# PJLab-ADG/DetZero

Measured on AMD Instinct MI355X. Metric: LiDAR frames/sec (160k pts, 0.1m voxels), higher is better.
Workload: dtype f32 as f16 pairs (hi+lo, 22-bit significand; 3 f16 MFMA per product, f32 accumulate)

## Files before the change

### detzero_amd/csrc/common.h

```cpp
#pragma once
#include <hip/hip_runtime.h>
#include <stdint.h>
#include <stdio.h>

#include "../../include/detzero_hip.h"

namespace dz {

void set_error(const char *fmt, ...);

#define DZ_CHECK_ARG(cond, ...)                 \
    do {                                        \
        if (!(cond)) {                          \
            dz::set_error(__VA_ARGS__);         \
            return DZ_ERR_INVALID;              \
        }                                       \
    } while (0)

#define DZ_HIP(expr)                                                                     \
    do {                                                                                 \
        hipError_t _e = (expr);                                                          \
        if (_e != hipSuccess) {                                                          \
            dz::set_error("%s failed: %s (%s:%d)", #expr, hipGetErrorString(_e), __FILE__, __LINE__); \
            return DZ_ERR_HIP;                                                           \
        }                                                                                \
    } while (0)

#define DZ_LAUNCH_CHECK()                                                                \
    do {                                                                                 \
        hipError_t _e = hipGetLastError();                                               \
        if (_e != hipSuccess) {                                                          \
            dz::set_error("kernel launch failed: %s (%s:%d)", hipGetErrorString(_e), __FILE__, __LINE__); \
            return DZ_ERR_HIP;                                                           \
        }                                                                                \
    } while (0)

static inline int ceil_div(long a, long b) { return (int)((a + b - 1) / b); }

static inline int tile_masks_words(int cap) { return (cap / 32 + 1 + 3) & ~3; }
static inline size_t align_up(size_t x, size_t a) { return (x + a - 1) / a * a; }

static inline int stream_grid(long work_items, int block) {
    long g = (work_items + block - 1) / block;
    if (g < 1) g = 1;
    if (g > 2048) g = 2048;
    return (int)g;
}

constexpr int DZ_MAX_DEVICES = 32;
struct PerDeviceFlags { bool v[DZ_MAX_DEVICES] = {}; };
static inline int reserve_lds(const void *kernel, int bytes, PerDeviceFlags &done, const char *who) {
    int dev = 0;
    if (hipGetDevice(&dev) != hipSuccess) { set_error("%s: hipGetDevice failed", who); return DZ_ERR_HIP; }
    if (dev >= 0 && dev < DZ_MAX_DEVICES && done.v[dev]) return DZ_OK;
    if (hipFuncSetAttribute(kernel, hipFuncAttributeMaxDynamicSharedMemorySize, bytes) != hipSuccess) {
        set_error("%s: cannot reserve %d bytes of LDS on device %d", who, bytes, dev);
        return DZ_ERR_HIP;
    }
    if (dev >= 0 && dev < DZ_MAX_DEVICES) done.v[dev] = true;
    return DZ_OK;
}
static inline int device_cus() {
    static int cus[DZ_MAX_DEVICES] = {};
// ... 85 lines not shown
```

### detzero_amd/csrc/conv3x3_h.hip

```cpp
#include "hgemm.h"

namespace dz {

constexpr int C3_TW = 32, C3_KC = 32;
constexpr int C3_ROW_U4 = C3_KC / 4 + 1;
constexpr int C3_PXW = C3_TW + 2;
constexpr int C3_NS = 3;
using v2u = __attribute__((ext_vector_type(2))) unsigned int;

constexpr int C3_NT = 512;
template <int BC>
struct C3Cfg {
    static constexpr int PT = 2;
    static constexpr int WC = BC >= 64 ? 2 : 1;
    static constexpr int WP = C3_NT / 64 / WC;
    static constexpr int TH = WP * PT;
    static constexpr int CT = BC / (32 * WC);
    static constexpr int PXH = TH + 2, PX_ROWS = C3_PXW * PXH, PX_PIECES = PX_ROWS * (C3_KC / 4);
    static constexpr int PXPT = (PX_PIECES + C3_NT - 1) / C3_NT;
    static constexpr int W_PIECES = BC * (C3_KC / 4);
    static constexpr int WPT = (W_PIECES + C3_NT - 1) / C3_NT;
    static constexpr int W_U4 = BC * C3_ROW_U4;
    static constexpr int LDS_MAIN_BYTES = (PX_ROWS * C3_ROW_U4 + 2 * W_U4) * 16;
    static constexpr int SG = 4;
// ... 21 lines not shown
    const int ntn = p.cout_pad / BC, nty = ny;
    const int *const tlist = p.in_tiles;
    const int npx = tlist ? tlist[0] : p.batch * tiles_x * tiles_y;
    const int xcd = blockIdx.x & 7, jloc = blockIdx.x >> 3, nj = gridDim.x >> 3;
    const int grp = (pair0 + jloc % nty) / ntn;
    const int n0 = ((pair0 + jloc % nty) % ntn) * BC;
    const int per_xcd = (npx + 7) >> 3;
    const int band_lo = xcd * per_xcd, band_hi = min(npx, band_lo + per_xcd);
    const int tstep = nj / nty;
    int tile = band_lo + jloc / nty;
    if (tstep == 0 || tile >= band_hi) return;

    const srsrc_t prsrc = make_srsrc(p.in, in_bytes);
    const srsrc_t crsrc = make_srsrc(p.w, w_bytes);
    int x0, y0, b;
    auto tile_id = [&](int t) {
        if (!tlist) return t;
        const int *ptr = tlist + 2 + t;
        int id;
        asm volatile("s_load_dword %0, %1, 0x0\n\ts_waitcnt lgkmcnt(0)" : "=&s"(id) : "s"(ptr) : "memory");
        return id;
    };
    auto tile_origin = [&](int t, int &ox, int &oy, int &ob) {
        ox = (t % tiles_x) * C3_TW;
        oy = ((t / tiles_x) % tiles_y) * C3_TH;
        ob = t / (tiles_x * tiles_y);
    };
    struct TileGeo { unsigned int base; int rows, cols; };
    auto tile_geo = [&](int t) {
        int ox, oy, ob;
        tile_origin(t, ox, oy, ob);
        TileGeo g;
        if constexpr (SPARSE) g.base = (unsigned int)((ob * p.in_hp + oy + p.in_off) * p.in_wp + ox + p.in_off);
        else g.base = (unsigned int)((((long)(ob * p.in_hp + oy + p.in_off) * p.in_wp + ox + p.in_off) * p.in_cstride + p.in_coff + grp * p.cin) * 4);
        g.rows = p.in_hp - (oy + p.in_off);
        g.cols = p.in_wp - (ox + p.in_off);
        return g;
    };
    int id_cur = tile_id(tile), id_next = id_cur;
    TileGeo geo = tile_geo(id_cur), geo_next = geo;
    const int prow = tid / (C3_KC / 4), pq = tid % (C3_KC / 4);
    bool has_next = tile + tstep < band_hi;
    unsigned int cvoff[WPT];
#pragma unroll
    for (int i = 0; i < WPT; ++i) {
        const int idx = tid + i * C3_NT;
// ... 360 lines not shown
```

### detzero_amd/csrc/pair16.hip

```cpp
#include "hgemm.h"

namespace dz {

template <class M>
__global__ void k_pair16_from_f32(const float *__restrict__ src, long rows, int c_src, int c_dst, uint4 *__restrict__ dst) {
    const int groups = c_dst / 8;
    const long total = rows * groups;
    for (long idx = (long)blockIdx.x * blockDim.x + threadIdx.x; idx < total; idx += (long)gridDim.x * blockDim.x) {
        const long r = idx / groups;
        const int g = (int)(idx % groups);
        float v[8];
#pragma unroll
        for (int e = 0; e < 8; ++e) v[e] = (g * 8 + e < c_src) ? src[r * c_src + g * 8 + e] : 0.f;
        const float a[4] = {v[0], v[1], v[2], v[3]}, b[4] = {v[4], v[5], v[6], v[7]};
        uint2 h0, l0, h1, l1;
        split4<M>(a, h0, l0);
        split4<M>(b, h1, l1);
        dst[idx * 2] = make_uint4(h0.x, h0.y, h1.x, h1.y);
        dst[idx * 2 + 1] = make_uint4(l0.x, l0.y, l1.x, l1.y);
    }
}

template <class M>
__global__ void k_pair16_to_f32(const uint4 *__restrict__ src, long rows, int c, float *__restrict__ dst) {
// ... 85 lines not shown
        bev[idx * 2 + 1] = zip(l0, l1);
    }
}

__global__ __launch_bounds__(256) void k_bev_row_index(const uint32_t *__restrict__ bitmap, const uint32_t *__restrict__ prefix, LevelGeom lg, int pad,
                                                       int feat_rows, int2 *__restrict__ idx) {
    const int hp = lg.h + 2 * pad, wp = lg.w + 2 * pad;
    const long total = (long)lg.b * hp * wp;
    for (long pix = (long)blockIdx.x * blockDim.x + threadIdx.x; pix < total; pix += (long)gridDim.x * blockDim.x) {
        const int xp = (int)(pix % wp), yp = (int)((pix / wp) % hp), b = (int)(pix / ((long)wp * hp));
        const int x = xp - pad, y = yp - pad;
        int r0 = -1, r1 = -1;
        if ((unsigned)x < (unsigned)lg.w && (unsigned)y < (unsigned)lg.h) {
            r0 = bitmap_find(bitmap, prefix, lg.key(b, 0, y, x));
            r1 = bitmap_find(bitmap, prefix, lg.key(b, 1, y, x));
            if (r0 >= feat_rows) r0 = -1;
            if (r1 >= feat_rows) r1 = -1;
        }
        idx[pix] = make_int2(r0, r1);
    }
}

constexpr int BEV_DCAP = 8;
__global__ __launch_bounds__(256) void k_bev_tile_mind(const int2 *__restrict__ idx, int batch, int hp, int wp, int ho, int wo, int tiles_y, int tiles_x,
                                                       unsigned char *__restrict__ mind) {
    constexpr int R = BEV_DCAP - 1, SH = 8 + 2 * R, SW = 32 + 2 * R;
    __shared__ unsigned char occ[SH][SW + 2];
    __shared__ int tile_min;
    const int t = blockIdx.x;
    const int tx = t % tiles_x, ty = (t / tiles_x) % tiles_y, b = t / (tiles_x * tiles_y);
    const int y0 = ty * 8 - R, x0 = tx * 32 - R;
    if (threadIdx.x == 0) tile_min = BEV_DCAP;
    for (int k = threadIdx.x; k < SH * SW; k += 256) {
        const int ry = k / SW, rx = k - ry * SW;
        const int y = y0 + ry, x = x0 + rx;
        unsigned char o = 0;
        if ((unsigned)y < (unsigned)ho && (unsigned)x < (unsigned)wo) {
            const int2 v = idx[((size_t)b * hp + y + 1) * wp + x + 1];
            o = (v.x >= 0 || v.y >= 0) ? 1 : 0;
        }
        occ[ry][rx] = o;
    }
    __syncthreads();
    const int py = threadIdx.x >> 5, px = threadIdx.x & 31;
    int d = BEV_DCAP;
    if (ty * 8 + py < ho && tx * 32 + px < wo) {
        const int cy = py + R, cx = px + R;
        if (occ[cy][cx]) d = 0;
        else {
            for (int r = 1; r <= R && d == BEV_DCAP; ++r) {
                bool hit = false;
                for (int k = -r; k <= r; ++k)
                    hit |= occ[cy - r][cx + k] | occ[cy + r][cx + k] | occ[cy + k][cx - r] | occ[cy + k][cx + r];
                if (hit) d = r;
            }
        }
    }
    atomicMin(&tile_min, d);
    __syncthreads();
    if (threadIdx.x == 0) mind[t] = (unsigned char)tile_min;
}

__global__ __launch_bounds__(1024) void k_bev_tile_compact(const unsigned char *__restrict__ mind, int n, int *__restrict__ lists, int stride) {
    __shared__ int part[1024];
    const int tid = threadIdx.x, need = (int)blockIdx.x + 2;
    int *const list = lists + (size_t)blockIdx.x * stride;
    const int per = (n + 1023) / 1024, lo = min(n, tid * per), hi = min(n, lo + per);
    int c = 0;
    for (int i = lo; i < hi; ++i) c += mind[i] < need;
    part[tid] = c;
    __syncthreads();
    for (int d = 1; d < 1024; d <<= 1) {
        const int v = tid >= d ? part[tid - d] : 0;
        __syncthreads();
        part[tid] += v;
        __syncthreads();
    }
    const int total = part[1023];
    int occ = part[tid] - c, emp = lo - occ;
    for (int i = lo; i < hi; ++i) {
        if (mind[i] < need) list[2 + occ++] = i;
        else list[2 + total + emp++] = i;
    }
    if (tid == 0) { list[0] = total; list[1] = n - total; }
}

template <class M>
__global__ __launch_bounds__(256) void k_bev_fill_tiles(const int *__restrict__ list, int tiles_y, int tiles_x, int ho, int wo, const float *__restrict__ shift,
                                                        int relu, int cout, float *__restrict__ out, int out_hp, int out_wp, int out_cstride, int out_coff,
                                                        const float *__restrict__ zero_resp) {
    const int n_occ = list[0], n_emp = list[1];
    if ((int)blockIdx.x >= n_emp) return;
    const int t = list[2 + n_occ + blockIdx.x];
    const int tx = t % tiles_x, ty = (t / tiles_x) % tiles_y, b = t / (tiles_x * tiles_y);
    const int groups = cout / 8;
    for (int k = threadIdx.x; k < 8 * 32 * groups; k += 256) {
        const int g = k % groups, px = k / groups, r = px / 32, c = px % 32;
        const int y = ty * 8 + r, x = tx * 32 + c;
        if (y >= ho || x >= wo) continue;
        uint4 *dst = reinterpret_cast<uint4 *>(out + (((size_t)b * out_hp + y + 1) * out_wp + x + 1) * out_cstride + out_coff + g * 8);
        if (zero_resp) {
            const uint4 *src = reinterpret_cast<const uint4 *>(zero_resp + (((size_t)(y + 1)) * out_wp + x + 1) * cout + g * 8);
            dst[0] = src[0];
            dst[1] = src[1];
            continue;
        }
        float v0[4], v1[4];
#pragma unroll
        for (int e = 0; e < 4; ++e) {
            const float a = shift ? shift[g * 8 + e] : 0.f, bb = shift ? shift[g * 8 + 4 + e] : 0.f;
            v0[e] = relu ? fmaxf(a, 0.f) : a;
            v1[e] = relu ? fmaxf(bb, 0.f) : bb;
        }
        uint2 h0, l0, h1, l1;
        split4<M>(v0, h0, l0);
        split4<M>(v1, h1, l1);
        dst[0] = make_uint4(h0.x, h0.y, h1.x, h1.y);
        dst[1] = make_uint4(l0.x, l0.y, l1.x, l1.y);
    }
}

}

using namespace dz;

extern "C" {

size_t dz_bev_tile_list_words(int batch, int ho, int wo) { return (size_t)batch * ceil_div(ho, 8) * ceil_div(wo, 32) + 2; }

int dz_bev_tile_list(const int *idx, int batch, int hp, int wp, int ho, int wo, int nlists, int *lists, unsigned char *mind_ws, void *stream_) {
    hipStream_t stream = (hipStream_t)stream_;
    DZ_CHECK_ARG(idx && lists && mind_ws && batch > 0 && ho > 0 && wo > 0 && hp >= ho + 2 && wp >= wo + 2 && nlists >= 1 && nlists < BEV_DCAP,
                 "dz_bev_tile_list: bad argument (1 <= nlists <= %d)", BEV_DCAP - 1);
    const int ty = ceil_div(ho, 8), tx = ceil_div(wo, 32), n = batch * ty * tx;
    hipLaunchKernelGGL(k_bev_tile_mind, dim3(n), dim3(256), 0, stream, reinterpret_cast<const int2 *>(idx), batch, hp, wp, ho, wo, ty, tx, mind_ws);
    hipLaunchKernelGGL(k_bev_tile_compact, dim3(nlists), dim3(1024), 0, stream, mind_ws, n, lists, (int)dz_bev_tile_list_words(batch, ho, wo));
    DZ_LAUNCH_CHECK();
    return DZ_OK;
}

int dz_bev_fill_empty_tiles(const int *list, int batch, int ho, int wo, const float *shift, int relu, int cout, float *out, int out_hp, int out_wp,
                            int out_cstride, int out_coff, const float *zero_resp, int math, void *stream_) {
    hipStream_t stream = (hipStream_t)stream_;
    DZ_CHECK_ARG(list && out && batch > 0 && ho > 0 && wo > 0 && cout > 0 && cout % 8 == 0 && out_cstride % 8 == 0 && out_coff % 8 == 0 &&
                 out_hp >= ho + 2 && out_wp >= wo + 2, "dz_bev_fill_empty_tiles: bad argument");
    DZ_CHECK_ARG(math == DZ_MATH_F16X2 || math == DZ_MATH_BF16X2 || math == DZ_MATH_F16, "dz_bev_fill_empty_tiles: math %d is not a split mode", math);
    const int ty = ceil_div(ho, 8), tx = ceil_div(wo, 32), n = batch * ty * tx;
    if (math == DZ_MATH_BF16X2)
        hipLaunchKernelGGL(k_bev_fill_tiles<MathBF16>, dim3(n), dim3(256), 0, stream, list, ty, tx, ho, wo, shift, relu, cout, out, out_hp, out_wp, out_cstride,
                           out_coff, zero_resp);
    else
        hipLaunchKernelGGL(k_bev_fill_tiles<MathF16>, dim3(n), dim3(256), 0, stream, list, ty, tx, ho, wo, shift, relu, cout, out, out_hp, out_wp, out_cstride,
                           out_coff, zero_resp);
    DZ_LAUNCH_CHECK();
    return DZ_OK;
}

int dz_bev_row_index(const uint32_t *bitmap, const uint32_t *prefix, int batch, int d, int h, int w, int layout, int pad, int feat_rows, int *idx,
                     void *stream_) {
    hipStream_t stream = (hipStream_t)stream_;
    DZ_CHECK_ARG(bitmap && prefix && idx && batch > 0 && h > 0 && w > 0 && pad >= 0 && feat_rows >= 0, "dz_bev_row_index: bad argument");
    if (d != 2) { set_error("dz_bev_row_index: %d z slabs (the sparse-input convolution reads exactly 2)", d); return DZ_ERR_UNSUPPORTED; }
    DZ_CHECK_ARG(layout == DZ_LAYOUT_LINEAR || layout == DZ_LAYOUT_BRICK, "dz_bev_row_index: bad layout %d", layout);
    const LevelGeom lg = make_level(batch, d, h, w, layout);
    const long total = (long)batch * (h + 2 * pad) * (w + 2 * pad);
    hipLaunchKernelGGL(k_bev_row_index, dim3(stream_grid(total, 256)), dim3(256), 0, stream, bitmap, prefix, lg, pad, feat_rows, reinterpret_cast<int2 *>(idx));
    DZ_LAUNCH_CHECK();
    return DZ_OK;
}

int dz_pair16_from_f32(const float *src, long rows, int c_src, int c_dst, int math, float *dst, void *stream_) {
    hipStream_t stream = (hipStream_t)stream_;
    DZ_CHECK_ARG(rows >= 0 && c_src >= 1 && c_dst >= c_src && c_dst % 8 == 0, "dz_pair16_from_f32: bad sizes");
    DZ_CHECK_ARG(math == DZ_MATH_F16X2 || math == DZ_MATH_BF16X2, "dz_pair16_from_f32: math %d is not a split mode", math);
    if (rows == 0) return DZ_OK;
    DZ_CHECK_ARG(src && dst, "dz_pair16_from_f32: null pointer");
// ... 72 lines not shown
```

### detzero_amd/det_modules.py

```python
import collections
import contextlib
import os
from functools import partial

import numpy as np
import torch
import torch.nn as nn

from . import ops, range_audit
from .lib import DetZeroHipError
from .range_audit import RangeAudit

PACKED_TABLES = bool(os.environ.get('DZ_TUNE_PACKED_TABLES'))

K3, S1, P1 = (3, 3, 3), (1, 1, 1), (1, 1, 1)


def _inference_only(module):
    if module.training:
        raise DetZeroHipError('%s: only the inference path is implemented on the HIP backend '
                              '(call .eval()); training is out of scope' % type(module).__name__)


def fold_bn(bn, conv_bias=None):
# ... 795 lines not shown
                CACHE_GEN[0] += 1
        if torch.cuda.is_current_stream_capturing():
            cache.pin(key)
        elif torch.device(dev).type == 'cuda':
            users.setdefault(key, set()).add(torch.cuda.current_stream(dev))
        return outs

    def _level_convs(self, li, lvl, x, xh, xw, xc, batch, dev, sparse_in=None, out_last=None):
        convs = lvl['convs']
        bufs = None
        tiles = zero = None
        audit = range_audit.active()
        e_in, e_mid = self._e('encoded'), self._e('spatial_features_2d')
        if sparse_in is not None and li == 0 and SKIP_EMPTY_TILES:
            nl = min(len(convs), 6) if all(cv['stride'] == 1 for cv in convs) else 1
            key = ('zero_resp', xh, xw, int(self.math), str(dev), int(batch), e_in, e_mid)
            if nl > 1 and key not in lvl and torch.cuda.is_current_stream_capturing():
                nl = 1
                if not getattr(self, '_warned_capture_nl1', False):
                    self._warned_capture_nl1 = True
                    import warnings
                    warnings.warn('BaseBEVBackbone: graph capture of a %d-frame pass without an eager pass of the same size before it - empty tiles '
                                  'are skipped at the first layer only (run one eager pass first to skip them in all six)' % batch)
            tiles = ops.bev_tile_list(sparse_in[1], xh, xw, nl)
            zero = self._zero_response(lvl, xh, xw, sparse_in[0].shape[1], dev, batch) if nl > 1 else None
        for ci, cv in enumerate(convs):
            s = cv['stride']
            oh, ow = (xh + 2 - 3) // s + 1, (xw + 2 - 3) // s + 1
            if bufs is None:
                bufs = [bordered_zeros('bev2d.l%d.%d' % (li, k), (batch, oh + 2, ow + 2, cv['cout']), dev) for k in range(2)]
            y = out_last if (out_last is not None and ci == len(convs) - 1) else bufs[ci % 2]
            if sparse_in is not None and li == 0 and ci == 0:
                rows, ridx = sparse_in
                wz, scz, shz = self._p(cv, e_in, e_mid, key='w_zmajor')
                conv_layer(rows, (xh + 2, xw + 2), wz, scz, shz, True, y, (oh + 2, ow + 2),
                           cin=cv['cin'], in_cstride=xc, ksize=3, stride=s, in_off=0, out_cstride=cv['cout'],
                           out_d=(1, 1), ho=oh, wo=ow, batch=batch, math=self.math, in_rowidx=ridx, in_row_channels=rows.shape[1],
                           in_rows=rows.shape[0], in_tiles=tiles[0] if tiles is not None else None)
                if tiles is not None:
                    ops.bev_fill_empty_tiles(tiles[0], batch, oh, ow, shz, True, cv['cout'], y, self.math)
            else:
                tl = tiles[ci] if (tiles is not None and ci < tiles.shape[0]) else None
                wc, scc, shc = self._p(cv, e_in if (li == 0 and ci == 0) else e_mid, e_mid)
                conv_layer(x, (xh + 2, xw + 2), wc, scc, shc, True, y, (oh + 2, ow + 2),
                           cin=cv['cin'], in_cstride=xc, ksize=3, stride=s, in_off=0, out_cstride=cv['cout'],
                           out_d=(1, 1), ho=oh, wo=ow, batch=batch, math=self.math, in_tiles=tl, w_limb3=self._l3(cv))
                if tl is not None:
# ... 430 lines not shown
```

### detzero_amd/lib.py

```python
import ctypes
import os

import torch

_HERE = os.path.dirname(os.path.abspath(__file__))
LIB_PATH = os.path.join(_HERE, 'libdetzero_hip.so')


ERR_INVALID, ERR_WORKSPACE, ERR_HIP, ERR_UNSUPPORTED = -1, -2, -3, -4


class DetZeroHipError(RuntimeError):
    pass


c_int, c_float, c_size_t, c_void_p, c_double = ctypes.c_int, ctypes.c_float, ctypes.c_size_t, ctypes.c_void_p, ctypes.c_double
c_longlong = ctypes.c_longlong
_I3 = c_int * 3
_F3 = c_float * 3
_F6 = c_float * 6
_I8 = c_int * 8


class Conv2dDesc(ctypes.Structure):
# ... 92 lines not shown
                                        c_void_p, c_void_p, c_void_p, c_int, c_void_p, c_int, c_int, c_void_p]),
    'dz_spconv_tiles_variant': (ctypes.c_char_p, [c_int, c_int]),
    'dz_spconv_x_tile_rows': (c_int, [c_int, c_int]),
    'dz_spconv_x_window_rows': (c_int, [c_int, c_int]),
    'dz_spconv_x_windows_words': (c_size_t, [c_int, c_int]),
    'dz_spconv_x_windows': (c_int, [c_void_p, c_int, c_void_p, c_int, c_void_p, c_void_p, c_void_p, c_void_p]),
    'dz_build_neighbors_packed_x': (c_int, [c_void_p, c_void_p, c_int, c_void_p, c_void_p, c_int, c_int, c_int, c_int, c_void_p, c_void_p, c_int,
                                            c_void_p, c_void_p, c_void_p, c_void_p]),
    'dz_spconv_forward_split_x': (c_int, [c_void_p, c_int, c_int, c_void_p, c_void_p, c_void_p, c_int, c_int, c_void_p, c_void_p, c_void_p, c_void_p,
                                          c_void_p, c_int, c_void_p, c_int, c_int, c_void_p]),
    'dz_spconv_x_variant': (ctypes.c_char_p, [c_int, c_int]),
    'dz_spconv_forward_x_f32': (c_int, [c_void_p, c_int, c_int, c_void_p, c_void_p, c_void_p, c_int, c_int, c_void_p, c_void_p, c_void_p, c_void_p,
                                        c_void_p, c_int, c_void_p, c_int, c_void_p]),
    'dz_spconv_x_f32_window_rows': (c_int, [c_int, c_int]),
    'dz_spconv_x_f32_variant': (ctypes.c_char_p, [c_int, c_int]),
    'dz_spconv_forward_x_limb3': (c_int, [c_void_p, c_int, c_int, c_void_p, c_void_p, c_void_p, c_int, c_int, c_void_p, c_void_p, c_void_p, c_void_p,
                                          c_void_p, c_int, c_void_p, c_int, c_void_p]),
    'dz_spconv_x_limb3_window_rows': (c_int, [c_int, c_int]),
    'dz_spconv_x_limb3_variant': (ctypes.c_char_p, [c_int, c_int]),
    'dz_spconv_forward_limb3': (c_int, [c_void_p, c_int, c_int, c_void_p, c_void_p, c_int, c_int, c_void_p, c_void_p, c_void_p, c_void_p,
                                        c_void_p, c_int, c_void_p, c_int, c_void_p]),
    'dz_spconv_limb3_tile_rows': (c_int, [c_int, c_int]),
    'dz_spconv_limb3_variant': (ctypes.c_char_p, [c_int, c_int]),
    'dz_bev_tile_list_words': (c_size_t, [c_int, c_int, c_int]),
    'dz_bev_tile_list': (c_int, [c_void_p, c_int, c_int, c_int, c_int, c_int, c_int, c_void_p, c_void_p, c_void_p]),
    'dz_bev_fill_empty_tiles': (c_int, [c_void_p, c_int, c_int, c_int, c_void_p, c_int, c_int, c_void_p, c_int, c_int, c_int, c_int, c_void_p, c_int, c_void_p]),
    'dz_bev_row_index': (c_int, [c_void_p, c_void_p, c_int, c_int, c_int, c_int, c_int, c_int, c_int, c_void_p, c_void_p]),
    'dz_sparse_to_bev_split': (c_int, [c_void_p, c_void_p, c_void_p, c_int, c_int, c_int, c_int, c_int, c_int, c_void_p,
                                       c_void_p]),
    'dz_sparse_to_bev_split_dense': (c_int, [c_void_p, c_int, c_void_p, c_void_p, c_int, c_int, c_int, c_int, c_int, c_int, c_int, c_void_p,
                                             c_void_p]),
    'dz_conv2d_forward_split': (c_int, [ctypes.POINTER(Conv2dDesc), c_int, c_int, c_void_p]),
    'dz_conv2d_variant_split': (ctypes.c_char_p, [ctypes.POINTER(Conv2dDesc), c_int]),
    'dz_conv3x3_limb3_forward': (c_int, [ctypes.POINTER(Conv2dDesc), c_void_p]),
    'dz_conv3x3_limb3_supported': (c_int, [ctypes.POINTER(Conv2dDesc)]),
    'dz_conv3x3_limb3_variant': (ctypes.c_char_p, [ctypes.POINTER(Conv2dDesc)]),
    'dz_spconv_variant_split': (ctypes.c_char_p, [c_int, c_int]),
    'dz_spconv_variant_split_arm': (ctypes.c_char_p, [c_int, c_int, c_int, c_int, c_size_t]),
    'dz_spconv_variant_split_packed': (ctypes.c_char_p, [c_int, c_int]),
    'dz_xattn_folded_supported': (c_int, [c_int, c_int, c_int]),
    'dz_xattn_folded_workspace_bytes': (ctypes.c_size_t, [c_int, c_int]),
    'dz_xattn_folded': (c_int, [c_void_p] * 6 + [c_int] * 5 + [ctypes.c_float, c_void_p, ctypes.c_size_t, c_void_p, c_void_p]),
    'dz_roi_bev_features': (c_int, [c_void_p, c_int, c_void_p, ctypes.c_long, ctypes.c_long, c_int, c_int, c_int] + [ctypes.c_float] * 4 + [c_int, c_void_p, c_void_p]),
    'dz_linear_splitk_workspace_bytes': (ctypes.c_size_t, [c_int, c_int, c_int]),
    'dz_linear_forward_splitk': (c_int, [c_void_p, c_int, c_int, c_int, c_void_p, c_int, c_int, c_void_p, c_void_p, c_int, c_void_p, c_int, c_int, c_void_p,
                                         ctypes.c_size_t, c_void_p]),
    'dz_mha_core_split': (c_int, [c_void_p, c_void_p, c_void_p, c_void_p, c_int, c_int, c_int, c_int, ctypes.c_float, c_void_p, c_int, c_void_p]),
    'dz_pdv_sa_pool_supported': (c_int, [c_int] * 7),
    'dz_pdv_sa_pool': (c_int, [c_void_p, c_int, c_int, c_void_p, c_void_p, c_int, c_void_p, c_void_p, c_int, c_void_p, c_void_p, c_int,
# ... 146 lines not shown
```

### detzero_amd/ops.py

```python
import ctypes
import os
from typing import Callable, NamedTuple, Optional

import numpy as np
import torch

from . import lib as L


def _dev():
    return torch.device('cuda', torch.cuda.current_device())


def _ws(nbytes):
    return torch.empty((max(int(nbytes), 256),), dtype=torch.uint8, device=_dev())


def grid_size_of(pc_range, voxel_size):
    r = np.asarray(pc_range, dtype=np.float32)
    return np.round((r[3:6] - r[0:3]) / np.array(voxel_size)).astype(np.int64)


def voxelize_hard_nosync(points, pc_range, voxel_size, max_points, max_voxels, xy_range_mask=False):
    lib = L.load()
# ... 427 lines not shown
        launch()
    else:
        m = out_level.num_active()
        pairs = table_pairs(nbr, m)
        flops = 2.0 * pairs * cin * cout
        n_in = in_level.num_active() if in_level is not None else m
        nbytes = 4.0 * (n_in * cin + m * cout + nbr.kvol * cin * cout + (m * cout if residual is not None else 0)) + 8.0 * pairs
        PROFILER.wrap(route.variant(cin, cout).decode(), flops, nbytes, launch)
    return out


def bev_row_index(level, feat_rows, pad=1):
    lib = L.load()
    d, h, w = level.shape
    idx = torch.empty((level.batch, h + 2 * pad, w + 2 * pad, 2), dtype=torch.int32, device=level.coords.device)
    rc = lib.dz_bev_row_index(L.ptr(level.bitmap), L.ptr(level.prefix), level.batch, d, h, w, level.layout, pad, int(feat_rows), L.ptr(idx), L.stream())
    L.check(rc, 'dz_bev_row_index')
    return idx


def bev_tile_list(ridx, ho, wo, nlists=1):
    lib = L.load()
    b, hp, wp, _ = ridx.shape
    n = lib.dz_bev_tile_list_words(b, int(ho), int(wo))
    lst = torch.empty((int(nlists), n), dtype=torch.int32, device=ridx.device)
    ws = torch.empty((n,), dtype=torch.uint8, device=ridx.device)
    L.check(lib.dz_bev_tile_list(L.ptr(ridx), b, hp, wp, int(ho), int(wo), int(nlists), L.ptr(lst), L.ptr(ws), L.stream()), 'dz_bev_tile_list')
    return lst


def bev_fill_empty_tiles(tiles, batch, ho, wo, shift, relu, cout, out, math, zero_resp=None):
    lib = L.load()
    L.check(lib.dz_bev_fill_empty_tiles(L.ptr(tiles), int(batch), int(ho), int(wo), L.ptr(shift), 1 if relu else 0, int(cout), L.ptr(out), out.shape[1],
                                        out.shape[2], out.shape[3], 0, L.ptr(zero_resp), int(math), L.stream()), 'dz_bev_fill_empty_tiles')


BEV_DENSE = not os.environ.get('DZ_BEV_SCATTER')


def sparse_to_bev(feats, level, c, pad=1, out=None, math=0):
    lib = L.load()
    d, h, w = level.shape
    if out is None:
        out = torch.empty((level.batch, h + 2 * pad, w + 2 * pad, c * d), dtype=torch.float32, device=feats.device)
    if math and d == 2 and c % 8 == 0 and BEV_DENSE:
        rc = lib.dz_sparse_to_bev_split_dense(L.ptr(feats), feats.shape[0], L.ptr(level.bitmap), L.ptr(level.prefix), level.batch, c, d, h, w, level.layout,
                                              pad, L.ptr(out), L.stream())
        L.check(rc, 'dz_sparse_to_bev_split_dense')
        return out
    out.zero_()
    fn = lib.dz_sparse_to_bev_split if math else lib.dz_sparse_to_bev
    rc = fn(L.ptr(feats), L.ptr(level.coords), L.ptr(level.d_m), level.cap, c, d, h, w, pad, L.ptr(out), L.stream())
    L.check(rc, 'dz_sparse_to_bev')
    return out


MATH_MODES = {'f32': 0, 'f16x2': 1, 'bf16x2': 2, 'f16': 3}
# ... 181 lines not shown
def conv2d(desc_kwargs, math=0, out_f32=False, tiles=None, f32_engine=None):
    lib = L.load()
    if f32_engine not in (None,) + DENSE_F32_ENGINES:
        raise L.DetZeroHipError('unknown fp32 dense engine %r (%s)' % (f32_engine, ' | '.join(DENSE_F32_ENGINES)))
    limb3 = f32_engine == 'bf16x3' and not math
    d = _conv2d_desc(desc_kwargs)

    def launch():
        if limb3:
            L.check(lib.dz_conv3x3_limb3_forward(ctypes.byref(d), L.stream()), 'dz_conv3x3_limb3_forward')
        elif math:
            L.check(lib.dz_conv2d_forward_split(ctypes.byref(d), int(math), 1 if out_f32 else 0, L.stream()), 'dz_conv2d_forward_split')
        else:
            L.check(lib.dz_conv2d_forward(ctypes.byref(d), L.stream()), 'dz_conv2d_forward')
    if PROFILER is None:
        launch()
        return
    m = d.batch * d.ho * d.wo
    taps = d.kh * d.kw
    cout = sum(d.g_cout[i] for i in range(d.groups))
    flops = 2.0 * m * taps * d.cin * cout
    nbytes = 4.0 * (m * d.cin * (1 if d.phase_groups else d.groups) + m * cout + taps * d.cin * d.cout_pad * d.groups)
    if tiles is not None:
        n_run, n_skip = (int(v) for v in tiles[:2].tolist())
        share = n_run / float(max(n_run + n_skip, 1))
        flops *= share
        nbytes = 4.0 * (share * (m * d.cin + m * cout) + taps * d.cin * d.cout_pad * d.groups)
    if limb3:
        name = lib.dz_conv3x3_limb3_variant(ctypes.byref(d)).decode()
    else:
        name = (lib.dz_conv2d_variant_split(ctypes.byref(d), 1 if out_f32 else 0) if math else lib.dz_conv2d_variant(ctypes.byref(d))).decode()
    PROFILER.wrap(name, flops, nbytes, launch)


def linear(x, w, scale, shift, relu, cout, out=None, group_shift=None, group_rows=0):
    lib = L.load()
    L.require_cuda(x, w, scale, shift, group_shift)
    rows, cin = x.shape
    cout_pad = w.shape[1]
    if out is None:
        out = torch.empty((rows, cout), dtype=torch.float32, device=x.device)
    rc = lib.dz_linear_forward(L.ptr(x), rows, cin, x.stride(0), L.ptr(w), cout, cout_pad, L.ptr(scale),
                               L.ptr(shift), L.ptr(group_shift), int(group_rows), 1 if relu else 0, L.ptr(out),
                               out.stride(0), L.stream())
    L.check(rc, 'dz_linear_forward')
    return out


# ... 748 lines not shown
```

### include/detzero_hip.h

```cpp
#ifndef DETZERO_HIP_H
#define DETZERO_HIP_H

#include <stddef.h>
#include <stdint.h>

#ifdef __cplusplus
extern "C" {
#endif

#define DZ_OK 0
#define DZ_ERR_INVALID (-1)
#define DZ_ERR_WORKSPACE (-2)
#define DZ_ERR_HIP (-3)
#define DZ_ERR_UNSUPPORTED (-4)

const char *dz_version(void);
const char *dz_last_error(void);
int dz_device_cu_count(void);


size_t dz_voxelize_hard_workspace_bytes(int n, int gx, int gy, int gz, int max_points);
int dz_voxelize_hard(const float *points, int n, int c, const float *h_range6, const float *h_vsize3,
                     const int *h_grid3, int xy_range_mask, int max_points, int max_voxels, float *voxels,
                     int *coords_zyx, int *num_points, int *d_num_voxels, void *ws, size_t ws_bytes,
// ... 118 lines not shown
                                int h, int w, int *nbr_packed, uint32_t *tile_masks, int tile_rows, int *windows, int *nbr_sorted,
                                int *perm, void *stream);
int dz_spconv_forward_split_x(const float *in, int in_rows, int cin, const int *nbr_packed, const int *perm, int *windows, int tile_rows,
                              int cap_out, const int *d_m_out, const float *w, const float *scale, const float *shift,
                              const float *residual, int relu, float *out, int cout, int math, void *stream);
const char *dz_spconv_x_variant(int cin, int cout);
int dz_spconv_forward_x_f32(const float *in, int in_rows, int cin, const int *nbr_packed, const int *perm, int *windows, int tile_rows,
                            int cap_out, const int *d_m_out, const float *w, const float *scale, const float *shift,
                            const float *residual, int relu, float *out, int cout, void *stream);
int dz_spconv_x_f32_window_rows(int cin, int cout);
const char *dz_spconv_x_f32_variant(int cin, int cout);
int dz_spconv_forward_x_limb3(const float *in, int in_rows, int cin, const int *nbr_packed, const int *perm, int *windows, int tile_rows,
                              int cap_out, const int *d_m_out, const float *w, const float *scale, const float *shift,
                              const float *residual, int relu, float *out, int cout, void *stream);
int dz_spconv_x_limb3_window_rows(int cin, int cout);
const char *dz_spconv_x_limb3_variant(int cin, int cout);
int dz_spconv_forward_limb3(const float *in, int in_rows, int cin, const int *nbr, const uint32_t *tile_masks, int kvol, int cap_out,
                            const int *d_m_out, const float *w_limb, const float *scale, const float *shift, const float *residual,
                            int relu, float *out, int cout, void *stream);
int dz_spconv_limb3_tile_rows(int cin, int cout);
const char *dz_spconv_limb3_variant(int cin, int cout);
int dz_bev_row_index(const uint32_t *bitmap, const uint32_t *prefix, int batch, int d, int h, int w, int layout, int pad, int feat_rows,
                     int *idx, void *stream);
size_t dz_bev_tile_list_words(int batch, int ho, int wo);
int dz_bev_tile_list(const int *idx, int batch, int hp, int wp, int ho, int wo, int nlists, int *lists, unsigned char *mind_ws, void *stream);
int dz_bev_fill_empty_tiles(const int *list, int batch, int ho, int wo, const float *shift, int relu, int cout, float *out, int out_hp, int out_wp,
                            int out_cstride, int out_coff, const float *zero_resp, int math, void *stream);
int dz_sparse_to_bev_split(const float *feats, const int *coords, const int *d_m, int cap, int c, int d, int h,
                           int w, int pad, float *bev, void *stream);
int dz_sparse_to_bev_split_dense(const float *feats, int feat_rows, const uint32_t *bitmap, const uint32_t *prefix, int batch, int c,
                                 int d, int h, int w, int layout, int pad, float *bev, void *stream);
int dz_conv2d_forward_split(const dz_conv2d_desc *h_desc, int math, int out_f32, void *stream);
const char *dz_conv2d_variant_split(const dz_conv2d_desc *h_desc, int out_f32);
int dz_conv3x3_limb3_forward(const dz_conv2d_desc *h_desc, void *stream);
int dz_conv3x3_limb3_supported(const dz_conv2d_desc *h_desc);
const char *dz_conv3x3_limb3_variant(const dz_conv2d_desc *h_desc);
int dz_linear_forward_split(const float *x, long rows, int cin, int x_stride, const float *w, int cout, int cout_pad, const float *scale,
                            const float *shift, const float *group_shift, int group_rows, int relu, float *y, int y_stride, int math,
                            int out_f32, int group_max, void *stream);
const char *dz_spconv_variant_split(int cin, int cout);
const char *dz_spconv_variant_split_arm(int cin, int cout, int kvol, int has_tile_masks, size_t nbr_bytes);
const char *dz_spconv_variant_split_packed(int cin, int cout);
int dz_xattn_folded_supported(int lq, int e, int heads);
size_t dz_xattn_folded_workspace_bytes(int b, int lk);
int dz_xattn_folded(const float *q, const float *mem, const uint8_t *key_padding_mask, const float *wk_oi, const float *wv_io, const float *bv,
                    int b, int lq, int lk, int e, int heads, float scale, float *workspace, size_t workspace_bytes, float *out, void *stream);
int dz_mlp_chain_forward(const float *x, long rows, const float *wa, const float *sa, const float *ba, const float *group_shift, int ldg, int group_rows,
                         const float *wb, const float *sb, const float *bb, const float *wk, const float *bk, const float *wv, const float *bv,
                         float *mem, float *k, float *v, int math, void *stream);
int dz_pointnet3_forward(const float *x, long rows, const float *w1, const float *s1, const float *b1, const float *w2, const float *s2,
// ... 214 lines not shown
```

Baseline: 1182.

## Replace fixed BEV tile grid skip with per-band greedy tile cover and span fills

Instead of skipping only fixed 32-wide grid tiles that are empty, each 8-row band is planned with a greedy cover that places 32-wide tiles starting at the first busy column, so fewer conv tiles are launched. The remaining empty gaps are emitted as spans and filled by a persistent grid-stride kernel with deeper vectorized stores. Conv3x3 tiles gain packed (batch, row, x) entries with arbitrary x origins. This adds planning complexity, packing limits on size and width, and a separate grid list for other consumers.

```diff
diff --git a/detzero_amd/csrc/common.h b/detzero_amd/csrc/common.h
--- a/detzero_amd/csrc/common.h
+++ b/detzero_amd/csrc/common.h
@@ -39,6 +39,10 @@
 
 static inline int tile_masks_words(int cap) { return (cap / 32 + 1 + 3) & ~3; }
 static inline size_t align_up(size_t x, size_t a) { return (x + a - 1) / a * a; }
+
+constexpr int TILE_XY_MAX_B = 1 << 10, TILE_XY_MAX_TY = 1 << 9, TILE_XY_MAX_X = 1 << 12;
+__host__ __device__ static inline int tile_xy_pack(int b, int ty, int x) { return (int)(0x80000000u | ((unsigned)b << 21) | ((unsigned)ty << 12) | (unsigned)x); }
+__host__ __device__ static inline void tile_xy_unpack(int e, int &b, int &ty, int &x) { x = e & 0xFFF; ty = (e >> 12) & 0x1FF; b = (e >> 21) & 0x3FF; }
 
 static inline int stream_grid(long work_items, int block) {
     long g = (work_items + block - 1) / block;
diff --git a/detzero_amd/csrc/conv3x3_h.hip b/detzero_amd/csrc/conv3x3_h.hip
--- a/detzero_amd/csrc/conv3x3_h.hip
+++ b/detzero_amd/csrc/conv3x3_h.hip
@@ -67,6 +67,12 @@
         return id;
     };
     auto tile_origin = [&](int t, int &ox, int &oy, int &ob) {
+        if (tlist && t < 0) {
+            int ty;
+            tile_xy_unpack(t, ob, ty, ox);
+            oy = ty * C3_TH;
+            return;
+        }
         ox = (t % tiles_x) * C3_TW;
         oy = ((t / tiles_x) % tiles_y) * C3_TH;
         ob = t / (tiles_x * tiles_y);
diff --git a/detzero_amd/csrc/pair16.hip b/detzero_amd/csrc/pair16.hip
--- a/detzero_amd/csrc/pair16.hip
+++ b/detzero_amd/csrc/pair16.hip
@@ -131,101 +131,164 @@
 }
 
 constexpr int BEV_DCAP = 8;
-__global__ __launch_bounds__(256) void k_bev_tile_mind(const int2 *__restrict__ idx, int batch, int hp, int wp, int ho, int wo, int tiles_y, int tiles_x,
-                                                       unsigned char *__restrict__ mind) {
-    constexpr int R = BEV_DCAP - 1, SH = 8 + 2 * R, SW = 32 + 2 * R;
-    __shared__ unsigned char occ[SH][SW + 2];
-    __shared__ int tile_min;
-    const int t = blockIdx.x;
-    const int tx = t % tiles_x, ty = (t / tiles_x) % tiles_y, b = t / (tiles_x * tiles_y);
-    const int y0 = ty * 8 - R, x0 = tx * 32 - R;
-    if (threadIdx.x == 0) tile_min = BEV_DCAP;
-    for (int k = threadIdx.x; k < SH * SW; k += 256) {
-        const int ry = k / SW, rx = k - ry * SW;
-        const int y = y0 + ry, x = x0 + rx;
-        unsigned char o = 0;
-        if ((unsigned)y < (unsigned)ho && (unsigned)x < (unsigned)wo) {
-            const int2 v = idx[((size_t)b * hp + y + 1) * wp + x + 1];
-            o = (v.x >= 0 || v.y >= 0) ? 1 : 0;
-        }
-        occ[ry][rx] = o;
+constexpr int BEV_MAX_W = 1024;
+static inline __host__ __device__ int bev_slot_words(int tiles_x) { return 3 + tiles_x + tiles_x + 1; }
+
+__global__ __launch_bounds__(256) void k_bev_cover_plan(const int2 *__restrict__ idx, int hp, int wp, int ho, int wo, int tiles_y, int tiles_x, int nl,
+                                                        int *__restrict__ slots) {
+    __shared__ unsigned char vd[BEV_MAX_W];
+    __shared__ unsigned long long busy[BEV_DCAP - 2][BEV_MAX_W / 64];
+    const int tid = threadIdx.x, ty = blockIdx.x % tiles_y, b = blockIdx.x / tiles_y, y0 = ty * 8;
+    for (int k = tid; k < (BEV_DCAP - 2) * (BEV_MAX_W / 64); k += 256) (&busy[0][0])[k] = 0ull;
+    for (int x = tid; x < wo; x += 256) {
+        int v = BEV_DCAP - 1;
+        for (int r = -nl; r < 8 + nl; ++r) {
+            const int y = y0 + r;
+            if ((unsigned)y >= (unsigned)ho) continue;
+            const int2 e = idx[((size_t)b * hp + y + 1) * wp + x + 1];
+            if (e.x >= 0 || e.y >= 0) v = min(v, r < 0 ? -r : r > 7 ? r - 7 : 0);
+        }
+        vd[x] = (unsigned char)v;
     }
     __syncthreads();
-    const int py = threadIdx.x >> 5, px = threadIdx.x & 31;
-    int d = BEV_DCAP;
-    if (ty * 8 + py < ho && tx * 32 + px < wo) {
-        const int cy = py + R, cx = px + R;
-        if (occ[cy][cx]) d = 0;
-        else {
-            for (int r = 1; r <= R && d == BEV_DCAP; ++r) {
-                bool hit = false;
-                for (int k = -r; k <= r; ++k)
-                    hit |= occ[cy - r][cx + k] | occ[cy + r][cx + k] | occ[cy + k][cx - r] | occ[cy + k][cx + r];
-                if (hit) d = r;
+    const int wo64 = (wo + 63) & ~63;
+    for (int l = 1; l <= nl; ++l)
+        for (int x = tid; x < wo64; x += 256) {
+            bool bz = false;
+            if (x < wo)
+                for (int k = max(0, x - l); k <= min(wo - 1, x + l); ++k) bz |= vd[k] <= l;
+            const unsigned long long m = __ballot(bz);
+            if ((tid & 63) == 0) busy[l - 1][x >> 6] = m;
+        }
+    __syncthreads();
+    if (tid >= nl) return;
+    const unsigned long long *const bm = busy[tid];
+    int *const s = slots + ((size_t)blockIdx.x * nl + tid) * bev_slot_words(tiles_x);
+    const int nw = wo64 >> 6;
+    int n = 0, ns = 0, pos = 0;
+    for (;;) {
+        int w = pos >> 6, x = wo;
+        unsigned long long m = bm[w] & (~0ull << (pos & 63));
+        while (!m && ++w < nw) m = bm[w];
+        if (m) x = w * 64 + __ffsll(m) - 1;
+        if (x > pos) s[3 + tiles_x + ns++] = pos | (x << 16);
+        if (x >= wo) break;
+        s[3 + n++] = x;
+        pos = x + 32;
+        if (pos >= wo) break;
+    }
+    unsigned int gm = 0u;
+    for (int tx = 0; tx < tiles_x; ++tx) gm |= (unsigned int)(bm[tx >> 1] >> (32 * (tx & 1))) ? 1u << tx : 0u;
+    s[0] = n;
+    s[1] = ns;
+    s[2] = (int)gm;
+}
+
+__global__ __launch_bounds__(64) void k_bev_cover_compact(const int *__restrict__ slots, int n_bands, int tiles_y, int tiles_x, int nl, int *__restrict__ lists,
+                                                          int stride) {
+    const int lane = threadIdx.x, l = blockIdx.y, first = blockIdx.x * 64, sw = bev_slot_words(tiles_x);
+    auto slot = [&](int i) { return slots + ((size_t)i * nl + l) * sw; };
+    int before[3] = {0, 0, 0}, total[3] = {0, 0, 0};
+    for (int i = lane; i < n_bands; i += 64) {
+        const int *s = slot(i);
+        const int c[3] = {s[0], s[1], (int)__popc((unsigned int)s[2])};
+        for (int k = 0; k < 3; ++k) { total[k] += c[k]; if (i < first) before[k] += c[k]; }
+    }
+    for (int k = 0; k < 3; ++k)
+        for (int d = 32; d >= 1; d >>= 1) { total[k] += __shfl_xor(total[k], d); before[k] += __shfl_xor(before[k], d); }
+    const int me = first + lane;
+    const bool live = me < n_bands;
+    const int *const s = slot(live ? me : 0);
+    const int n = live ? s[0] : 0, ns = live ? s[1] : 0;
+    const unsigned int gm = live ? (unsigned int)s[2] : 0u;
+    int pre[3] = {n, ns, (int)__popc(gm)};
+    for (int k = 0; k < 3; ++k) {
+        for (int d = 1; d < 64; d <<= 1) { const int t = __shfl_up(pre[k], d); if (lane >= d) pre[k] += t; }
+        pre[k] += before[k];
+    }
+    int *const grid = lists + (size_t)l * stride, *const cover = grid + 2 + n_bands * tiles_x;
+    if (blockIdx.x == 0 && lane == 0) {
+        grid[0] = total[2];
+        grid[1] = n_bands * tiles_x - total[2];
+        cover[0] = total[0];
+        cover[1] = total[1];
+    }
+    if (!live) return;
+    const int b = me / tiles_y, ty = me % tiles_y;
+    int *o = cover + 2 + pre[0] - n;
+    for (int k = 0; k < n; ++k) o[k] = tile_xy_pack(b, ty, s[3 + k]);
+    o = cover + 2 + total[0] + 2 * (pre[1] - ns);
+    for (int k = 0; k < ns; ++k) {
+        const int sp = s[3 + tiles_x + k];
+        o[2 * k] = tile_xy_pack(b, ty, sp & 0xFFFF);
+        o[2 * k + 1] = sp >> 16;
+    }
+    int run = pre[2] - (int)__popc(gm);
+    for (int tx = 0; tx < tiles_x; ++tx) {
+        const int id = me * tiles_x + tx;
+        if ((gm >> tx) & 1u) grid[2 + run++] = id;
+        else grid[2 + total[2] + id - run] = id;
+    }
+}
+
+constexpr int FILL_DEPTH = 8;
+template <class M>
+__global__ __launch_bounds__(256) void k_bev_fill_spans(const int *__restrict__ list, int batch, int tiles_y, int tiles_x, int ho, int wo,
+                                                        const float *__restrict__ shift, int relu, int cout, float *__restrict__ out, int out_hp, int out_wp,
+                                                        int out_cstride, int out_coff, const float *__restrict__ zero_resp) {
+    const int n_run = list[0], n_fill = min(list[1], batch * tiles_y * (tiles_x + 1));
+    if (n_fill <= 0) return;
+    const int *const ent = list + 2 + n_run;
+    const bool xy = ent[0] < 0;
+    const int lane = threadIdx.x & 63;
+    const int y8 = blockIdx.x & 7;
+    const int wave = __builtin_amdgcn_readfirstlane((int)((blockIdx.x >> 3) * 4 + (threadIdx.x >> 6))), nwaves = (gridDim.x >> 3) * 4;
+    const int ppp = cout / 4;
+    const int nseg = (wo + 63) / 64;
+    for (int u = wave; u < n_fill * nseg; u += nwaves) {
+        const int i = u / nseg, seg = u - i * nseg;
+        int b, ty, xs, xe;
+        if (xy) {
+            tile_xy_unpack(ent[2 * i], b, ty, xs);
+            xe = ent[2 * i + 1];
+        } else {
+            const int t = ent[i];
+            xs = (t % tiles_x) * 32, xe = min(xs + 32, wo), ty = (t / tiles_x) % tiles_y, b = t / (tiles_x * tiles_y);
+        }
+        const int y = ty * 8 + y8;
+        if ((unsigned)b >= (unsigned)batch || y >= ho || xs < 0 || xe > wo) continue;
+        xs += seg * 64;
+        if (xs >= xe) continue;
+        xe = min(xe, xs + 64);
+        const int np = (xe - xs) * ppp;
+        float *const drow = out + (((size_t)b * out_hp + y + 1) * out_wp + xs + 1) * out_cstride + out_coff;
+        const uint4 *const srow = zero_resp ? reinterpret_cast<const uint4 *>(zero_resp + ((size_t)(y + 1) * out_wp + xs + 1) * cout) : nullptr;
+        for (int p0 = lane; p0 < np; p0 += 64 * FILL_DEPTH) {
+            uint4 v[FILL_DEPTH];
+#pragma unroll
+            for (int k = 0; k < FILL_DEPTH; ++k) {
+                const int p = p0 + 64 * k;
+                if (p >= np) continue;
+                if (srow) { v[k] = srow[p]; continue; }
+                const int g = (p % ppp) >> 1;
+                float v0[4], v1[4];
+#pragma unroll
+                for (int e = 0; e < 4; ++e) {
+                    const float a = shift ? shift[g * 8 + e] : 0.f, bb = shift ? shift[g * 8 + 4 + e] : 0.f;
+                    v0[e] = relu ? fmaxf(a, 0.f) : a;
+                    v1[e] = relu ? fmaxf(bb, 0.f) : bb;
+                }
+                uint2 h0, l0, h1, l1;
+                split4<M>(v0, h0, l0);
+                split4<M>(v1, h1, l1);
+                v[k] = (p & 1) ? make_uint4(l0.x, l0.y, l1.x, l1.y) : make_uint4(h0.x, h0.y, h1.x, h1.y);
             }
-        }
-    }
-    atomicMin(&tile_min, d);
-    __syncthreads();
-    if (threadIdx.x == 0) mind[t] = (unsigned char)tile_min;
-}
-
-__global__ __launch_bounds__(1024) void k_bev_tile_compact(const unsigned char *__restrict__ mind, int n, int *__restrict__ lists, int stride) {
-    __shared__ int part[1024];
-    const int tid = threadIdx.x, need = (int)blockIdx.x + 2;
-    int *const list = lists + (size_t)blockIdx.x * stride;
-    const int per = (n + 1023) / 1024, lo = min(n, tid * per), hi = min(n, lo + per);
-    int c = 0;
-    for (int i = lo; i < hi; ++i) c += mind[i] < need;
-    part[tid] = c;
-    __syncthreads();
-    for (int d = 1; d < 1024; d <<= 1) {
-        const int v = tid >= d ? part[tid - d] : 0;
-        __syncthreads();
-        part[tid] += v;
-        __syncthreads();
-    }
-    const int total = part[1023];
-    int occ = part[tid] - c, emp = lo - occ;
-    for (int i = lo; i < hi; ++i) {
-        if (mind[i] < need) list[2 + occ++] = i;
-        else list[2 + total + emp++] = i;
-    }
-    if (tid == 0) { list[0] = total; list[1] = n - total; }
-}
-
-template <class M>
-__global__ __launch_bounds__(256) void k_bev_fill_tiles(const int *__restrict__ list, int tiles_y, int tiles_x, int ho, int wo, const float *__restrict__ shift,
-                                                        int relu, int cout, float *__restrict__ out, int out_hp, int out_wp, int out_cstride, int out_coff,
-                                                        const float *__restrict__ zero_resp) {
-    const int n_occ = list[0], n_emp = list[1];
-    if ((int)blockIdx.x >= n_emp) return;
-    const int t = list[2 + n_occ + blockIdx.x];
-    const int tx = t % tiles_x, ty = (t / tiles_x) % tiles_y, b = t / (tiles_x * tiles_y);
-    const int groups = cout / 8;
-    for (int k = threadIdx.x; k < 8 * 32 * groups; k += 256) {
-        const int g = k % groups, px = k / groups, r = px / 32, c = px % 32;
-        const int y = ty * 8 + r, x = tx * 32 + c;
-        if (y >= ho || x >= wo) continue;
-        uint4 *dst = reinterpret_cast<uint4 *>(out + (((size_t)b * out_hp + y + 1) * out_wp + x + 1) * out_cstride + out_coff + g * 8);
-        if (zero_resp) {
-            const uint4 *src = reinterpret_cast<const uint4 *>(zero_resp + (((size_t)(y + 1)) * out_wp + x + 1) * cout + g * 8);
-            dst[0] = src[0];
-            dst[1] = src[1];
-            continue;
-        }
-        float v0[4], v1[4];
-#pragma unroll
-        for (int e = 0; e < 4; ++e) {
-            const float a = shift ? shift[g * 8 + e] : 0.f, bb = shift ? shift[g * 8 + 4 + e] : 0.f;
-            v0[e] = relu ? fmaxf(a, 0.f) : a;
-            v1[e] = relu ? fmaxf(bb, 0.f) : bb;
-        }
-        uint2 h0, l0, h1, l1;
-        split4<M>(v0, h0, l0);
-        split4<M>(v1, h1, l1);
-        dst[0] = make_uint4(h0.x, h0.y, h1.x, h1.y);
-        dst[1] = make_uint4(l0.x, l0.y, l1.x, l1.y);
+#pragma unroll
+            for (int k = 0; k < FILL_DEPTH; ++k) {
+                const int p = p0 + 64 * k;
+                if (p < np) *reinterpret_cast<uint4 *>(drow + (size_t)(p / ppp) * out_cstride + (p % ppp) * 4) = v[k];
+            }
+        }
     }
 }
 
@@ -235,32 +298,43 @@
 
 extern "C" {
 
-size_t dz_bev_tile_list_words(int batch, int ho, int wo) { return (size_t)batch * ceil_div(ho, 8) * ceil_div(wo, 32) + 2; }
-
-int dz_bev_tile_list(const int *idx, int batch, int hp, int wp, int ho, int wo, int nlists, int *lists, unsigned char *mind_ws, void *stream_) {
-    hipStream_t stream = (hipStream_t)stream_;
-    DZ_CHECK_ARG(idx && lists && mind_ws && batch > 0 && ho > 0 && wo > 0 && hp >= ho + 2 && wp >= wo + 2 && nlists >= 1 && nlists < BEV_DCAP,
-                 "dz_bev_tile_list: bad argument (1 <= nlists <= %d)", BEV_DCAP - 1);
-    const int ty = ceil_div(ho, 8), tx = ceil_div(wo, 32), n = batch * ty * tx;
-    hipLaunchKernelGGL(k_bev_tile_mind, dim3(n), dim3(256), 0, stream, reinterpret_cast<const int2 *>(idx), batch, hp, wp, ho, wo, ty, tx, mind_ws);
-    hipLaunchKernelGGL(k_bev_tile_compact, dim3(nlists), dim3(1024), 0, stream, mind_ws, n, lists, (int)dz_bev_tile_list_words(batch, ho, wo));
-    DZ_LAUNCH_CHECK();
-    return DZ_OK;
-}
-
-int dz_bev_fill_empty_tiles(const int *list, int batch, int ho, int wo, const float *shift, int relu, int cout, float *out, int out_hp, int out_wp,
-                            int out_cstride, int out_coff, const float *zero_resp, int math, void *stream_) {
+static inline int bev_bands(int batch, int ho) { return batch * ceil_div(ho, 8); }
+size_t dz_bev_tile_cover_offset(int batch, int ho, int wo) { return (size_t)bev_bands(batch, ho) * ceil_div(wo, 32) + 2; }
+size_t dz_bev_tile_cover_words(int batch, int ho, int wo) {
+    const size_t n = bev_bands(batch, ho), tx = ceil_div(wo, 32);
+    return dz_bev_tile_cover_offset(batch, ho, wo) + 2 + n * tx + 2 * n * (tx + 1);
+}
+size_t dz_bev_tile_cover_ws_words(int batch, int ho, int wo, int nlists) { return (size_t)bev_bands(batch, ho) * nlists * bev_slot_words(ceil_div(wo, 32)); }
+
+int dz_bev_tile_cover(const int *idx, int batch, int hp, int wp, int ho, int wo, int nlists, int *lists, int *ws, void *stream_) {
+    hipStream_t stream = (hipStream_t)stream_;
+    DZ_CHECK_ARG(idx && lists && ws && batch > 0 && ho > 0 && wo > 0 && hp >= ho + 2 && wp >= wo + 2 && nlists >= 1 && nlists <= BEV_DCAP - 2,
+                 "dz_bev_tile_cover: bad argument (1 <= nlists <= %d)", BEV_DCAP - 2);
+    const int ty = ceil_div(ho, 8), tx = ceil_div(wo, 32), n = batch * ty;
+    DZ_CHECK_ARG(wo <= BEV_MAX_W && wo <= TILE_XY_MAX_X && ty <= TILE_XY_MAX_TY && batch <= TILE_XY_MAX_B,
+                 "dz_bev_tile_cover: %d frames of %d x %d pixels exceed the list entry (%d frames, %d rows, %d columns)", batch, ho, wo, TILE_XY_MAX_B,
+                 TILE_XY_MAX_TY * 8, BEV_MAX_W);
+    hipLaunchKernelGGL(k_bev_cover_plan, dim3(n), dim3(256), 0, stream, reinterpret_cast<const int2 *>(idx), hp, wp, ho, wo, ty, tx, nlists, ws);
+    hipLaunchKernelGGL(k_bev_cover_compact, dim3(ceil_div(n, 64), nlists), dim3(64), 0, stream, ws, n, ty, tx, nlists, lists,
+                       (int)dz_bev_tile_cover_words(batch, ho, wo));
+    DZ_LAUNCH_CHECK();
+    return DZ_OK;
+}
+
+int dz_bev_fill_spans(const int *list, int batch, int ho, int wo, const float *shift, int relu, int cout, float *out, int out_hp, int out_wp,
+                      int out_cstride, int out_coff, const float *zero_resp, int math, void *stream_) {
     hipStream_t stream = (hipStream_t)stream_;
     DZ_CHECK_ARG(list && out && batch > 0 && ho > 0 && wo > 0 && cout > 0 && cout % 8 == 0 && out_cstride % 8 == 0 && out_coff % 8 == 0 &&
-                 out_hp >= ho + 2 && out_wp >= wo + 2, "dz_bev_fill_empty_tiles: bad argument");
-    DZ_CHECK_ARG(math == DZ_MATH_F16X2 || math == DZ_MATH_BF16X2 || math == DZ_MATH_F16, "dz_bev_fill_empty_tiles: math %d is not a split mode", math);
-    const int ty = ceil_div(ho, 8), tx = ceil_div(wo, 32), n = batch * ty * tx;
+                 out_hp >= ho + 2 && out_wp >= wo + 2, "dz_bev_fill_spans: bad argument");
+    DZ_CHECK_ARG(math == DZ_MATH_F16X2 || math == DZ_MATH_BF16X2 || math == DZ_MATH_F16, "dz_bev_fill_spans: math %d is not a split mode", math);
+    const int ty = ceil_div(ho, 8), tx = ceil_div(wo, 32);
+    const dim3 grid((4 * device_cus() + 7) / 8 * 8);
     if (math == DZ_MATH_BF16X2)
-        hipLaunchKernelGGL(k_bev_fill_tiles<MathBF16>, dim3(n), dim3(256), 0, stream, list, ty, tx, ho, wo, shift, relu, cout, out, out_hp, out_wp, out_cstride,
-                           out_coff, zero_resp);
+        hipLaunchKernelGGL(k_bev_fill_spans<MathBF16>, grid, dim3(256), 0, stream, list, batch, ty, tx, ho, wo, shift, relu, cout, out, out_hp, out_wp,
+                           out_cstride, out_coff, zero_resp);
     else
-        hipLaunchKernelGGL(k_bev_fill_tiles<MathF16>, dim3(n), dim3(256), 0, stream, list, ty, tx, ho, wo, shift, relu, cout, out, out_hp, out_wp, out_cstride,
-                           out_coff, zero_resp);
+        hipLaunchKernelGGL(k_bev_fill_spans<MathF16>, grid, dim3(256), 0, stream, list, batch, ty, tx, ho, wo, shift, relu, cout, out, out_hp, out_wp,
+                           out_cstride, out_coff, zero_resp);
     DZ_LAUNCH_CHECK();
     return DZ_OK;
 }
diff --git a/detzero_amd/det_modules.py b/detzero_amd/det_modules.py
--- a/detzero_amd/det_modules.py
+++ b/detzero_amd/det_modules.py
@@ -841,7 +841,7 @@
                     import warnings
                     warnings.warn('BaseBEVBackbone: graph capture of a %d-frame pass without an eager pass of the same size before it - empty tiles '
                                   'are skipped at the first layer only (run one eager pass first to skip them in all six)' % batch)
-            tiles = ops.bev_tile_list(sparse_in[1], xh, xw, nl)
+            tiles = ops.bev_tile_cover(ops.bev_tile_list(sparse_in[1], xh, xw, nl), batch, xh, xw)
             zero = self._zero_response(lvl, xh, xw, sparse_in[0].shape[1], dev, batch) if nl > 1 else None
         for ci, cv in enumerate(convs):
             s = cv['stride']
diff --git a/detzero_amd/lib.py b/detzero_amd/lib.py
--- a/detzero_amd/lib.py
+++ b/detzero_amd/lib.py
@@ -138,9 +138,11 @@
                                         c_void_p, c_int, c_void_p, c_int, c_void_p]),
     'dz_spconv_limb3_tile_rows': (c_int, [c_int, c_int]),
     'dz_spconv_limb3_variant': (ctypes.c_char_p, [c_int, c_int]),
-    'dz_bev_tile_list_words': (c_size_t, [c_int, c_int, c_int]),
-    'dz_bev_tile_list': (c_int, [c_void_p, c_int, c_int, c_int, c_int, c_int, c_int, c_void_p, c_void_p, c_void_p]),
-    'dz_bev_fill_empty_tiles': (c_int, [c_void_p, c_int, c_int, c_int, c_void_p, c_int, c_int, c_void_p, c_int, c_int, c_int, c_int, c_void_p, c_int, c_void_p]),
+    'dz_bev_tile_cover_words': (c_size_t, [c_int, c_int, c_int]),
+    'dz_bev_tile_cover_offset': (c_size_t, [c_int, c_int, c_int]),
+    'dz_bev_tile_cover_ws_words': (c_size_t, [c_int, c_int, c_int, c_int]),
+    'dz_bev_tile_cover': (c_int, [c_void_p, c_int, c_int, c_int, c_int, c_int, c_int, c_void_p, c_void_p, c_void_p]),
+    'dz_bev_fill_spans': (c_int, [c_void_p, c_int, c_int, c_int, c_void_p, c_int, c_int, c_void_p, c_int, c_int, c_int, c_int, c_void_p, c_int, c_void_p]),
     'dz_bev_row_index': (c_int, [c_void_p, c_void_p, c_int, c_int, c_int, c_int, c_int, c_int, c_int, c_void_p, c_void_p]),
     'dz_sparse_to_bev_split': (c_int, [c_void_p, c_void_p, c_void_p, c_int, c_int, c_int, c_int, c_int, c_int, c_void_p,
                                        c_void_p]),
diff --git a/detzero_amd/ops.py b/detzero_amd/ops.py
--- a/detzero_amd/ops.py
+++ b/detzero_amd/ops.py
@@ -473,17 +473,21 @@
 def bev_tile_list(ridx, ho, wo, nlists=1):
     lib = L.load()
     b, hp, wp, _ = ridx.shape
-    n = lib.dz_bev_tile_list_words(b, int(ho), int(wo))
+    n = lib.dz_bev_tile_cover_words(b, int(ho), int(wo))
     lst = torch.empty((int(nlists), n), dtype=torch.int32, device=ridx.device)
-    ws = torch.empty((n,), dtype=torch.uint8, device=ridx.device)
-    L.check(lib.dz_bev_tile_list(L.ptr(ridx), b, hp, wp, int(ho), int(wo), int(nlists), L.ptr(lst), L.ptr(ws), L.stream()), 'dz_bev_tile_list')
+    ws = torch.empty((lib.dz_bev_tile_cover_ws_words(b, int(ho), int(wo), int(nlists)),), dtype=torch.int32, device=ridx.device)
+    L.check(lib.dz_bev_tile_cover(L.ptr(ridx), b, hp, wp, int(ho), int(wo), int(nlists), L.ptr(lst), L.ptr(ws), L.stream()), 'dz_bev_tile_cover')
     return lst
 
 
+def bev_tile_cover(lists, batch, ho, wo):
+    return lists[:, L.load().dz_bev_tile_cover_offset(int(batch), int(ho), int(wo)):]
+
+
 def bev_fill_empty_tiles(tiles, batch, ho, wo, shift, relu, cout, out, math, zero_resp=None):
     lib = L.load()
-    L.check(lib.dz_bev_fill_empty_tiles(L.ptr(tiles), int(batch), int(ho), int(wo), L.ptr(shift), 1 if relu else 0, int(cout), L.ptr(out), out.shape[1],
-                                        out.shape[2], out.shape[3], 0, L.ptr(zero_resp), int(math), L.stream()), 'dz_bev_fill_empty_tiles')
+    L.check(lib.dz_bev_fill_spans(L.ptr(tiles), int(batch), int(ho), int(wo), L.ptr(shift), 1 if relu else 0, int(cout), L.ptr(out), out.shape[1],
+                                  out.shape[2], out.shape[3], 0, L.ptr(zero_resp), int(math), L.stream()), 'dz_bev_fill_spans')
 
 
 BEV_DENSE = not os.environ.get('DZ_BEV_SCATTER')
@@ -711,8 +715,7 @@
     flops = 2.0 * m * taps * d.cin * cout
     nbytes = 4.0 * (m * d.cin * (1 if d.phase_groups else d.groups) + m * cout + taps * d.cin * d.cout_pad * d.groups)
     if tiles is not None:
-        n_run, n_skip = (int(v) for v in tiles[:2].tolist())
-        share = n_run / float(max(n_run + n_skip, 1))
+        share = int(tiles[0]) / float(max(d.batch * (-(-d.ho // 8)) * (-(-d.wo // 32)), 1))
         flops *= share
         nbytes = 4.0 * (share * (m * d.cin + m * cout) + taps * d.cin * d.cout_pad * d.groups)
     if limb3:
diff --git a/include/detzero_hip.h b/include/detzero_hip.h
--- a/include/detzero_hip.h
+++ b/include/detzero_hip.h
@@ -164,10 +164,12 @@
 const char *dz_spconv_limb3_variant(int cin, int cout);
 int dz_bev_row_index(const uint32_t *bitmap, const uint32_t *prefix, int batch, int d, int h, int w, int layout, int pad, int feat_rows,
                      int *idx, void *stream);
-size_t dz_bev_tile_list_words(int batch, int ho, int wo);
-int dz_bev_tile_list(const int *idx, int batch, int hp, int wp, int ho, int wo, int nlists, int *lists, unsigned char *mind_ws, void *stream);
-int dz_bev_fill_empty_tiles(const int *list, int batch, int ho, int wo, const float *shift, int relu, int cout, float *out, int out_hp, int out_wp,
-                            int out_cstride, int out_coff, const float *zero_resp, int math, void *stream);
+size_t dz_bev_tile_cover_words(int batch, int ho, int wo);
+size_t dz_bev_tile_cover_offset(int batch, int ho, int wo);
+size_t dz_bev_tile_cover_ws_words(int batch, int ho, int wo, int nlists);
+int dz_bev_tile_cover(const int *idx, int batch, int hp, int wp, int ho, int wo, int nlists, int *lists, int *ws, void *stream);
+int dz_bev_fill_spans(const int *list, int batch, int ho, int wo, const float *shift, int relu, int cout, float *out, int out_hp, int out_wp,
+                      int out_cstride, int out_coff, const float *zero_resp, int math, void *stream);
 int dz_sparse_to_bev_split(const float *feats, const int *coords, const int *d_m, int cap, int c, int d, int h,
                            int w, int pad, float *bev, void *stream);
 int dz_sparse_to_bev_split_dense(const float *feats, int feat_rows, const uint32_t *bitmap, const uint32_t *prefix, int batch, int c,
```

After: 1196 (median of 6 runs). 1.2% higher.
